# tulip-control/polytope

Hardware: AMD Instinct MI355X
Metric: LP solves/sec (batched Chebyshev + redundancy) (higher is better)
Workload: dtype f64

## Files before the change

### polytope_amd/csrc/plp_lane_lp.hpp

```cpp
#pragma once
#include <math.h>

#if defined(__HIPCC__)
#include "plp_common.hpp"
#define PLP_LANE_FN __device__ __forceinline__
#else
#define PLP_LANE_FN static inline
namespace plp {
enum : int { ST_OPT = 0, ST_ITER = 1, ST_INFEAS = 2, ST_UNBND = 3, ST_NUM = 4 };
constexpr int ST_RETRY = 5;
constexpr double TOL_D = 1e-9, TOL_PIV = 1e-7, DEGEN_EPS = 1e-12;
constexpr int BLAND_AFTER = 6;
}
#endif

namespace plp {
namespace lane {

constexpr int LANE_MAX_ITERS = 48;
constexpr double LANE_TOL_D = 1e-11, LANE_TOL_PIV = 1e-11;
constexpr double LANE_M_NOISE = 64 * 2.220446049250313e-16;

struct Lp3 {
    double x0, x1, x2;
    int w0, w1, w2;
    int nact;
    int status;
    int iters;
    int ndeg;
};

PLP_LANE_FN void cross3(double a0, double a1, double a2, double b0, double b1, double b2, double& e0, double& e1,
                        double& e2) {
    e0 = fma(a1, b2, -(a2 * b1));
    e1 = fma(a2, b0, -(a0 * b2));
    e2 = fma(a0, b1, -(a1 * b0));
}

PLP_LANE_FN double dot3(double a0, double a1, double a2, double b0, double b1, double b2) {
    return fma(a2, b2, fma(a1, b1, a0 * b0));
}

template <class AnyF>
PLP_LANE_FN void proj1(const double c0, const double c1, const double c2, const double cn1, const double n0, const double n1,
                       const double n2, const double nn, double& d0, double& d1, double& d2, double& scale, AnyF ANY) {
    const double cn = dot3(c0, c1, c2, n0, n1, n2);
    d0 = fma(cn, n0, -(nn * c0));
    d1 = fma(cn, n1, -(nn * c1));
    d2 = fma(cn, n2, -(nn * c2));
    scale = nn;
    const double pn1 = fabs(d0) + fabs(d1) + fabs(d2);
    const bool small = (pn1 > 0.0) & (pn1 < 1e-4 * (nn * cn1));
    if (ANY(small)) {
        const double np_ = dot3(n0, n1, n2, d0, d1, d2);
        const double q0 = fma(nn, d0, -(np_ * n0)), q1 = fma(nn, d1, -(np_ * n1)), q2 = fma(nn, d2, -(np_ * n2));
        d0 = small ? q0 : d0;
        d1 = small ? q1 : d1;
        d2 = small ? q2 : d2;
        scale = small ? nn * nn : nn;
    }
}

constexpr double LANE_PAIR_SIN2 = 1e-10;

template <class RowF, class RatioF, class Ratio0F, class AnyF>
PLP_LANE_FN void walk3(Lp3& S, const double c0, const double c1, const double c2, const bool go, RowF ROWS, RatioF RATIO,
                       Ratio0F RATIO0, AnyF ANY, const bool warm = false) {
    if (!warm) {
        S.x0 = S.x1 = S.x2 = 0.0;
        S.w0 = S.w1 = S.w2 = -1;
        S.nact = 0;
        S.iters = 0;
        S.ndeg = 0;
    }
    S.status = go ? -1 : ST_OPT;
    const double cn1 = fabs(c0) + fabs(c1) + fabs(c2);
    if (go && !(cn1 > 0.0)) S.status = ST_OPT;
    if (!warm && ANY(S.status < 0)) {
        const bool step = S.status < 0;
        const double d0 = -c0, d1 = -c1, d2 = -c2;
        const double tolp = LANE_TOL_PIV * cn1;
        double bs = 1.0, bd = 0.0;
        int bi = -1;
        RATIO0(d0, d1, d2, tolp, bs, bd, bi);
        if (step) {
            S.iters = 1;
            if (bi < 0) {
                S.status = ST_UNBND;
            } else {
                const double t = bs / bd;
                S.x0 = fma(t, d0, 0.0);
                S.x1 = fma(t, d1, 0.0);
                S.x2 = fma(t, d2, 0.0);
                S.w0 = bi;
                S.nact = 1;
                S.ndeg = (t * cn1 <= DEGEN_EPS) ? 1 : 0;
            }
        }
    }
    while (ANY(S.status < 0)) {
        const bool run = S.status < 0;
        double d0 = -c0, d1 = -c1, d2 = -c2;
        double n00 = 0, n01 = 0, n02 = 0, n10 = 0, n11 = 0, n12 = 0, n20 = 0, n21 = 0, n22 = 0;
        if (ANY(run && S.nact >= 1)) {
            if (S.nact >= 1) ROWS(S.w0, n00, n01, n02);
            if (S.nact >= 2) ROWS(S.w1, n10, n11, n12);
            if (S.nact >= 3) ROWS(S.w2, n20, n21, n22);
        }
        bool stalled = false;
        double dscale = cn1;
        if (S.nact == 1) {
            const double nn = dot3(n00, n01, n02, n00, n01, n02);
            double sc;
            proj1(c0, c1, c2, cn1, n00, n01, n02, nn, d0, d1, d2, sc, ANY);
            dscale = sc * cn1;
        } else if (S.nact == 2) {
            double e0, e1, e2;
            cross3(n00, n01, n02, n10, n11, n12, e0, e1, e2);
            const double ce = dot3(c0, c1, c2, e0, e1, e2);
            d0 = -(ce * e0);
            d1 = -(ce * e1);
            d2 = -(ce * e2);
            dscale = dot3(e0, e1, e2, e0, e1, e2) * cn1;
            const double nn0 = dot3(n00, n01, n02, n00, n01, n02), nn1 = dot3(n10, n11, n12, n10, n11, n12);
            if (run && !(dot3(e0, e1, e2, e0, e1, e2) > LANE_PAIR_SIN2 * nn0 * nn1)) S.status = ST_RETRY;
        } else if (S.nact == 3) {
            d0 = d1 = d2 = 0.0;
        }
        {
            const double dn1 = fabs(d0) + fabs(d1) + fabs(d2);
            stalled = !(dn1 > LANE_TOL_D * dscale);
        }
        if (ANY(S.status < 0 && stalled)) {
            if (S.status < 0 && stalled) {
                if (S.nact == 0) {
                    S.status = ST_OPT;
                } else if (S.nact == 1) {
                    const double cn = dot3(c0, c1, c2, n00, n01, n02);
                    if (cn <= 0.0) S.status = ST_OPT;
                    else { S.nact = 0; d0 = -c0; d1 = -c1; d2 = -c2; }
                } else if (S.nact == 2) {
                    const double g00 = dot3(n00, n01, n02, n00, n01, n02), g11 = dot3(n10, n11, n12, n10, n11, n12);
                    const double g01 = dot3(n00, n01, n02, n10, n11, n12);
                    const double r0 = -dot3(c0, c1, c2, n00, n01, n02), r1 = -dot3(c0, c1, c2, n10, n11, n12);
                    const double l0 = fma(r0, g11, -(r1 * g01)), l1 = fma(r1, g00, -(r0 * g01));
                    const double w0 = 0.5 * (1.0 + g00), w1 = 0.5 * (1.0 + g11);
                    const double tol0 = LANE_TOL_D * g11 * w0 * cn1, tol1 = LANE_TOL_D * g00 * w1 * cn1;
                    if (l0 >= -tol0 && l1 >= -tol1) S.status = ST_OPT;
                    else {
                        const bool drop0 = l0 * w0 < l1 * w1;
                        if (drop0) { S.w0 = S.w1; n00 = n10; n01 = n11; n02 = n12; }
                        S.nact = 1;
                        double sc;
                        proj1(c0, c1, c2, cn1, n00, n01, n02, dot3(n00, n01, n02, n00, n01, n02), d0, d1, d2, sc, [](bool q) { return q; });
                    }
                } else {
                    double u00, u01, u02, u10, u11, u12, u20, u21, u22;
                    cross3(n10, n11, n12, n20, n21, n22, u00, u01, u02);
                    cross3(n20, n21, n22, n00, n01, n02, u10, u11, u12);
                    cross3(n00, n01, n02, n10, n11, n12, u20, u21, u22);
                    const double det = dot3(n00, n01, n02, u00, u01, u02);
                    const double g00 = dot3(n00, n01, n02, n00, n01, n02), g11 = dot3(n10, n11, n12, n10, n11, n12);
                    const double g22 = dot3(n20, n21, n22, n20, n21, n22);
                    if (!(det * det > 1e-18 * (g00 * g11 * g22))) {
                        S.status = ST_RETRY;
                    } else {
                        const double sg = det > 0.0 ? 1.0 : -1.0;
                        const double l0 = -sg * dot3(c0, c1, c2, u00, u01, u02);
                        const double l1 = -sg * dot3(c0, c1, c2, u10, u11, u12);
                        const double l2 = -sg * dot3(c0, c1, c2, u20, u21, u22);
                        const double a0 = l0 * (0.5 * (1.0 + g00)), a1 = l1 * (0.5 * (1.0 + g11)), a2 = l2 * (0.5 * (1.0 + g22));
                        const double tol = LANE_TOL_D * fabs(det) * cn1;
                        if (a0 >= -tol && a1 >= -tol && a2 >= -tol) S.status = ST_OPT;
                        else {
                            int j = 0;
                            double am = a0;
                            if (a1 < am) { am = a1; j = 1; }
                            if (a2 < am) { am = a2; j = 2; }
                            double gg;
                            if (j == 0) { d0 = -sg * u00; d1 = -sg * u01; d2 = -sg * u02; S.w0 = S.w1; S.w1 = S.w2; gg = g11 * g22; }
                            else if (j == 1) { d0 = -sg * u10; d1 = -sg * u11; d2 = -sg * u12; S.w1 = S.w2; gg = g22 * g00; }
                            else { d0 = -sg * u20; d1 = -sg * u21; d2 = -sg * u22; gg = g00 * g11; }
                            S.nact = 2;
                            if (!(dot3(d0, d1, d2, d0, d1, d2) > LANE_PAIR_SIN2 * gg)) S.status = ST_RETRY;
                        }
                    }
                }
            }
        }
        const bool step = S.status < 0;
        const double dn1 = fabs(d0) + fabs(d1) + fabs(d2);
        const double tolp = LANE_TOL_PIV * dn1;
        double bs = 1.0, bd = 0.0;
        int bi = -1;
        if (ANY(step)) RATIO(d0, d1, d2, S.x0, S.x1, S.x2, tolp, bs, bd, bi);
        if (step) {
            ++S.iters;
            if (bi < 0) {
                S.status = ST_UNBND;
            } else {
                const double t = bs / bd;
                S.x0 = fma(t, d0, S.x0);
                S.x1 = fma(t, d1, S.x1);
                S.x2 = fma(t, d2, S.x2);
                if (S.nact == 0) S.w0 = bi;
                else if (S.nact == 1) S.w1 = bi;
                else S.w2 = bi;
                S.nact += 1;
                S.ndeg = (t * dn1 <= DEGEN_EPS) ? S.ndeg + 1 : 0;
                if (S.ndeg >= BLAND_AFTER || S.iters >= LANE_MAX_ITERS) S.status = ST_RETRY;
            }
        }
    }
}

template <class RowF, class RatioF, class AnyF>
PLP_LANE_FN void walk3(Lp3& S, const double c0, const double c1, const double c2, const bool go, RowF ROWS, RatioF RATIO,
                       AnyF ANY, const bool warm = false) {
    walk3(S, c0, c1, c2, go, ROWS, RATIO,
          [&](double d0, double d1, double d2, double tolp, double& bs, double& bd, int& bi) {
              RATIO(d0, d1, d2, 0.0, 0.0, 0.0, tolp, bs, bd, bi);
          },
          ANY, warm);
}

struct Lp4 {
    double x0, x1, x2, x3;
    int w0, w1, w2, w3;
    int nact, status, iters, ndeg;
};

PLP_LANE_FN double dot4(double a0, double a1, double a2, double a3, double b0, double b1, double b2, double b3) {
    return fma(a3, b3, fma(a2, b2, fma(a1, b1, a0 * b0)));
}

PLP_LANE_FN void gcross4(double p0, double p1, double p2, double p3, double q0, double q1, double q2, double q3, double r0,
                         double r1, double r2, double r3, double& e0, double& e1, double& e2, double& e3) {
    const double m01 = fma(q0, r1, -(q1 * r0)), m02 = fma(q0, r2, -(q2 * r0)), m03 = fma(q0, r3, -(q3 * r0));
    const double m12 = fma(q1, r2, -(q2 * r1)), m13 = fma(q1, r3, -(q3 * r1)), m23 = fma(q2, r3, -(q3 * r2));
    e0 = fma(p1, m23, fma(-p2, m13, p3 * m12));
    e1 = -fma(p0, m23, fma(-p2, m03, p3 * m02));
    e2 = fma(p0, m13, fma(-p1, m03, p3 * m01));
    e3 = -fma(p0, m12, fma(-p1, m02, p2 * m01));
}

template <class RowF, class RatioF, class AnyF>
PLP_LANE_FN void walk4(Lp4& S, const double c0, const double c1, const double c2, const double c3, const bool go, RowF ROWS,
                       RatioF RATIO, AnyF ANY) {
    S.x0 = S.x1 = S.x2 = S.x3 = 0.0;
    S.w0 = S.w1 = S.w2 = S.w3 = -1;
    S.nact = 0;
    S.iters = 0;
    S.ndeg = 0;
    S.status = go ? -1 : ST_OPT;
    const double cn1 = fabs(c0) + fabs(c1) + fabs(c2) + fabs(c3);
    if (go && !(cn1 > 0.0)) S.status = ST_OPT;
    while (ANY(S.status < 0)) {
        const bool run = S.status < 0;
        bool dropped = false;
        double d0 = -c0, d1 = -c1, d2 = -c2, d3 = -c3;
        double n00 = 0, n01 = 0, n02 = 0, n03 = 0, n10 = 0, n11 = 0, n12 = 0, n13 = 0;
        double n20 = 0, n21 = 0, n22 = 0, n23 = 0, n30 = 0, n31 = 0, n32 = 0, n33 = 0;
        if (ANY(run && S.nact >= 1)) {
            if (S.nact >= 1) ROWS(S.w0, n00, n01, n02, n03);
            if (S.nact >= 2) ROWS(S.w1, n10, n11, n12, n13);
            if (S.nact >= 3) ROWS(S.w2, n20, n21, n22, n23);
            if (S.nact >= 4) ROWS(S.w3, n30, n31, n32, n33);
        }
        const double g00 = dot4(n00, n01, n02, n03, n00, n01, n02, n03), g11 = dot4(n10, n11, n12, n13, n10, n11, n12, n13);
        const double g22 = dot4(n20, n21, n22, n23, n20, n21, n22, n23);
        const double g01 = dot4(n00, n01, n02, n03, n10, n11, n12, n13), g02 = dot4(n00, n01, n02, n03, n20, n21, n22, n23);
        const double g12 = dot4(n10, n11, n12, n13, n20, n21, n22, n23);
        const double r0 = dot4(c0, c1, c2, c3, n00, n01, n02, n03), r1 = dot4(c0, c1, c2, c3, n10, n11, n12, n13);
        const double r2 = dot4(c0, c1, c2, c3, n20, n21, n22, n23);
        double det = 1.0, m0 = 0.0, m1 = 0.0, m2 = 0.0;
        if (S.nact == 1) {
            det = g00;
            m0 = r0;
        } else if (S.nact == 2) {
            det = fma(g00, g11, -(g01 * g01));
            m0 = fma(r0, g11, -(r1 * g01));
            m1 = fma(r1, g00, -(r0 * g01));
            if (run && !(det > LANE_PAIR_SIN2 * g00 * g11)) S.status = ST_RETRY;
        } else if (S.nact == 3) {
            const double A00 = fma(g11, g22, -(g12 * g12)), A01 = fma(g02, g12, -(g01 * g22)), A02 = fma(g01, g12, -(g02 * g11));
            const double A11 = fma(g00, g22, -(g02 * g02)), A12 = fma(g01, g02, -(g00 * g12)), A22 = fma(g00, g11, -(g01 * g01));
            det = fma(g00, A00, fma(g01, A01, g02 * A02));
            m0 = fma(A00, r0, fma(A01, r1, A02 * r2));
            m1 = fma(A01, r0, fma(A11, r1, A12 * r2));
            m2 = fma(A02, r0, fma(A12, r1, A22 * r2));
            if (run && !(det > 1e-16 * g00 * g11 * g22)) S.status = ST_RETRY;
        }
        bool twice = false;
        if (S.nact == 3) {
            double e0, e1, e2, e3;
            gcross4(n00, n01, n02, n03, n10, n11, n12, n13, n20, n21, n22, n23, e0, e1, e2, e3);
            const double ce = dot4(c0, c1, c2, c3, e0, e1, e2, e3);
            d0 = -(ce * e0);
            d1 = -(ce * e1);
            d2 = -(ce * e2);
            d3 = -(ce * e3);
        } else if (S.nact >= 1 && S.nact <= 2) {
            d0 = fma(m1, n10, fma(m0, n00, -(det * c0)));
            d1 = fma(m1, n11, fma(m0, n01, -(det * c1)));
            d2 = fma(m1, n12, fma(m0, n02, -(det * c2)));
            d3 = fma(m1, n13, fma(m0, n03, -(det * c3)));
            if (S.nact == 1) {
                const double nd = dot4(n00, n01, n02, n03, d0, d1, d2, d3);
                d0 = fma(g00, d0, -(nd * n00));
                d1 = fma(g00, d1, -(nd * n01));
                d2 = fma(g00, d2, -(nd * n02));
                d3 = fma(g00, d3, -(nd * n03));
            } else {
                const double dn = fabs(d0) + fabs(d1) + fabs(d2) + fabs(d3);
                twice = (dn > 0.0) & (dn < 1e-4 * (det * cn1));
                if (ANY(run && twice)) {
                    const double s0 = dot4(d0, d1, d2, d3, n00, n01, n02, n03), s1 = dot4(d0, d1, d2, d3, n10, n11, n12, n13);
                    const double k0 = fma(s0, g11, -(s1 * g01)), k1 = fma(s1, g00, -(s0 * g01));
                    const double q0 = fma(det, d0, -fma(k1, n10, k0 * n00)), q1 = fma(det, d1, -fma(k1, n11, k0 * n01));
                    const double q2 = fma(det, d2, -fma(k1, n12, k0 * n02)), q3 = fma(det, d3, -fma(k1, n13, k0 * n03));
                    d0 = twice ? q0 : d0;
                    d1 = twice ? q1 : d1;
                    d2 = twice ? q2 : d2;
                    d3 = twice ? q3 : d3;
                }
            }
        } else if (S.nact == 4) {
            d0 = d1 = d2 = d3 = 0.0;
        }
        const double dscale = (S.nact >= 1 && S.nact <= 3) ? ((S.nact == 1 || twice) ? det * det : det) * cn1 : cn1;
        const bool stalled = !(fabs(d0) + fabs(d1) + fabs(d2) + fabs(d3) > LANE_TOL_D * dscale);
        if (ANY(S.status < 0 && stalled)) {
            if (S.status < 0 && stalled) {
                const double w0 = 0.5 * (1.0 + g00), w1 = 0.5 * (1.0 + g11), w2 = 0.5 * (1.0 + g22);
                if (S.nact == 0) {
                    S.status = ST_OPT;
                } else if (S.nact <= 3) {
                    const double tol = LANE_TOL_D * det * cn1;
                    double f0 = 0.0, f1 = 0.0, f2 = 0.0;
                    if (S.nact == 2) {
                        f0 = fabs(r0 * g11) + fabs(r1 * g01);
                        f1 = fabs(r1 * g00) + fabs(r0 * g01);
                    } else if (S.nact == 3) {
                        const double B00 = fabs(g11 * g22) + g12 * g12, B01 = fabs(g02 * g12) + fabs(g01 * g22), B02 = fabs(g01 * g12) + fabs(g02 * g11);
                        const double B11 = fabs(g00 * g22) + g02 * g02, B12 = fabs(g01 * g02) + fabs(g00 * g12), B22 = fabs(g00 * g11) + g01 * g01;
                        f0 = B00 * fabs(r0) + B01 * fabs(r1) + B02 * fabs(r2);
                        f1 = B01 * fabs(r0) + B11 * fabs(r1) + B12 * fabs(r2);
                        f2 = B02 * fabs(r0) + B12 * fabs(r1) + B22 * fabs(r2);
                    }
                    const double a0 = -m0 * w0, a1 = S.nact >= 2 ? -m1 * w1 : 0.0, a2 = S.nact >= 3 ? -m2 * w2 : 0.0;
                    const double t0 = fmax(tol, LANE_M_NOISE * f0 * w0), t1 = fmax(tol, LANE_M_NOISE * f1 * w1), t2 = fmax(tol, LANE_M_NOISE * f2 * w2);
                    if (a0 >= -t0 && a1 >= -t1 && a2 >= -t2) {
                        S.status = ST_OPT;
                    } else {
                        int j = 0;
                        double am = a0 + t0;
                        if (a1 + t1 < am) { am = a1 + t1; j = 1; }
                        if (a2 + t2 < am) { am = a2 + t2; j = 2; }
                        if (j == 0) S.w0 = S.w1;
                        if (j <= 1) S.w1 = S.w2;
                        S.nact -= 1;
                        dropped = true;
                    }
                } else {
                    const double g33 = dot4(n30, n31, n32, n33, n30, n31, n32, n33);
                    const double w3 = 0.5 * (1.0 + g33);
                    double am = 0.0, bd0 = 0.0, bd1 = 0.0, bd2 = 0.0, bd3 = 0.0, dj_abs = 0.0;
                    int jbest = -1;
                    bool all_ok = true, singular = false;
#define PLP_W4_VERTEX(J, P, Q, R, NJ0, NJ1, NJ2, NJ3, WJ)                                                          \
                    {                                                                                                   \
                        double u0, u1, u2, u3;                                                                          \
                        gcross4(P##0, P##1, P##2, P##3, Q##0, Q##1, Q##2, Q##3, R##0, R##1, R##2, R##3, u0, u1, u2, u3); \
                        const double dj = dot4(NJ0, NJ1, NJ2, NJ3, u0, u1, u2, u3);                                     \
                        const double sg = dj > 0.0 ? 1.0 : -1.0;                                                        \
                        const double lj = -sg * dot4(c0, c1, c2, c3, u0, u1, u2, u3);                                   \
                        const double aj = lj * (WJ);                                                                    \
                        dj_abs = fabs(dj);                                                                              \
                        singular = singular | !(dj * dj > 1e-18 * (g00 * g11 * g22 * g33));                            \
                        all_ok = all_ok & (aj >= -(LANE_TOL_D * dj_abs * cn1));                                              \
                        const bool better = (jbest < 0) | (aj < am);                                                    \
                        am = better ? aj : am;                                                                          \
                        jbest = better ? (J) : jbest;                                                                   \
                        bd0 = better ? -sg * u0 : bd0;                                                                  \
                        bd1 = better ? -sg * u1 : bd1;                                                                  \
                        bd2 = better ? -sg * u2 : bd2;                                                                  \
                        bd3 = better ? -sg * u3 : bd3;                                                                  \
                    }
                    PLP_W4_VERTEX(0, n1, n2, n3, n00, n01, n02, n03, w0)
                    PLP_W4_VERTEX(1, n0, n2, n3, n10, n11, n12, n13, w1)
                    PLP_W4_VERTEX(2, n0, n1, n3, n20, n21, n22, n23, w2)
                    PLP_W4_VERTEX(3, n0, n1, n2, n30, n31, n32, n33, w3)
#undef PLP_W4_VERTEX
                    if (singular) S.status = ST_RETRY;
                    else if (all_ok) S.status = ST_OPT;
                    else {
                        d0 = bd0; d1 = bd1; d2 = bd2; d3 = bd3;
                        if (jbest == 0) S.w0 = S.w1;
                        if (jbest <= 1) S.w1 = S.w2;
                        if (jbest <= 2) S.w2 = S.w3;
                        S.nact = 3;
                    }
                }
            }
        }
        if (dropped) {
            ++S.iters;
            if (S.iters >= LANE_MAX_ITERS) S.status = ST_RETRY;
        }
        const bool step = (S.status < 0) & !dropped;
        const double dn1 = fabs(d0) + fabs(d1) + fabs(d2) + fabs(d3);
        const double tolp = LANE_TOL_PIV * dn1;
        double bs = 1.0, bd = 0.0;
        int bi = -1;
        if (ANY(step)) RATIO(d0, d1, d2, d3, S.x0, S.x1, S.x2, S.x3, tolp, bs, bd, bi);
        if (step) {
            ++S.iters;
            if (bi < 0) {
                S.status = ST_UNBND;
            } else {
                const double t = bs / bd;
                S.x0 = fma(t, d0, S.x0);
                S.x1 = fma(t, d1, S.x1);
                S.x2 = fma(t, d2, S.x2);
                S.x3 = fma(t, d3, S.x3);
                if (S.nact == 0) S.w0 = bi;
                else if (S.nact == 1) S.w1 = bi;
                else if (S.nact == 2) S.w2 = bi;
                else S.w3 = bi;
                S.nact += 1;
                S.ndeg = (t * dn1 <= DEGEN_EPS) ? S.ndeg + 1 : 0;
                if (S.ndeg >= BLAND_AFTER || S.iters >= LANE_MAX_ITERS) S.status = ST_RETRY;
            }
        }
    }
}

PLP_LANE_FN void ratio_row4(const double a0, const double a1, const double a2, const double a3, const double beta, const int i,
                            const double d0, const double d1, const double d2, const double d3, const double x0,
                            const double x1, const double x2, const double x3, const double tolp, double& bs, double& bd,
                            int& bi) {
    const double ad = dot4(a0, a1, a2, a3, d0, d1, d2, d3);
    const double ax = dot4(a0, a1, a2, a3, x0, x1, x2, x3);
    const double sl = fmax(beta - ax, 0.0);
    const bool better = (ad > tolp) & (sl * bd < bs * ad);
    bs = better ? sl : bs;
    bd = better ? ad : bd;
    bi = better ? i : bi;
}

PLP_LANE_FN void ratio_row(const double a0, const double a1, const double a2, const double beta, const int i, const double d0,
                           const double d1, const double d2, const double x0, const double x1, const double x2,
                           const double tolp, double& bs, double& bd, int& bi) {
    const double ad = dot3(a0, a1, a2, d0, d1, d2);
    const double ax = dot3(a0, a1, a2, x0, x1, x2);
    const double sl = fmax(beta - ax, 0.0);
    const bool better = (ad > tolp) & (sl * bd < bs * ad);
    bs = better ? sl : bs;
    bd = better ? ad : bd;
    bi = better ? i : bi;
}

PLP_LANE_FN void ratio_row0(const double a0, const double a1, const double a2, const double beta, const int i, const double d0,
                            const double d1, const double d2, const double tolp, double& bs, double& bd, int& bi) {
    const double ad = dot3(a0, a1, a2, d0, d1, d2);
    const double sl = fmax(beta, 0.0);
    const bool better = (ad > tolp) & (sl * bd < bs * ad);
    bs = better ? sl : bs;
    bd = better ? ad : bd;
    bi = better ? i : bi;
}

#ifndef PLP_LANE_CH
#define PLP_LANE_CH 4
#endif

PLP_LANE_FN void latch_row(const bool elig, const bool closer, const double sl, const double ad, const int i, double& bs,
                           double& bd, int& bi) {
#if defined(__HIP_DEVICE_COMPILE__) && !defined(PLP_LANE_SELECT_LATCH)
    const unsigned long long mask = __builtin_amdgcn_ballot_w64(elig) & __builtin_amdgcn_ballot_w64(closer);
    unsigned long long saved;
    asm("s_and_saveexec_b64 %[sv], %[m]\n\t"
        "v_mov_b64 %[bs], %[sl]\n\t"
        "v_mov_b64 %[bd], %[ad]\n\t"
        "v_mov_b32 %[bi], %[i]\n\t"
        "s_mov_b64 exec, %[sv]"
        : [bs] "+v"(bs), [bd] "+v"(bd), [bi] "+v"(bi), [sv] "=&s"(saved)
        : [m] "s"(mask), [sl] "v"(sl), [ad] "v"(ad), [i] "s"(i)
        : "scc");
#else
    const bool better = elig & closer;
    bs = better ? sl : bs;
    bd = better ? ad : bd;
    bi = better ? i : bi;
#endif
}

PLP_LANE_FN double relax_row(const bool at, double beta) {
#if defined(__HIP_DEVICE_COMPILE__) && !defined(PLP_LANE_SELECT_LATCH)
    const unsigned long long mask = __builtin_amdgcn_ballot_w64(at);
    unsigned long long saved;
    asm("s_and_saveexec_b64 %[sv], %[m]\n\t"
        "v_add_f64 %[b], %[b], %[c]\n\t"
        "s_mov_b64 exec, %[sv]"
        : [b] "+v"(beta), [sv] "=&s"(saved)
        : [m] "s"(mask), [c] "s"(0.1)
        : "scc");
    return beta;
#else
    return at ? beta + 0.1 : beta;
#endif
}

enum : int { RATIO_WALK = 0, RATIO_FIRST = 1, RATIO_AXIS = 2 };

template <int D, int LS, int MODE, bool RELAX>
PLP_LANE_FN void ratio_rows(const double* pA, const double* pbeta, const int i0, const int cnt, const int krv,
                            const double (&dv)[4], const double (&xv)[4], const int kax, const double dk, const double tolp,
                            double& bs, double& bd, int& bi) {
    static_assert(D >= 1 && D <= 4 && (D < 4 || MODE == RATIO_WALK), "R^4 has no peeled first pass");
    const double* ra = pA + i0 * D * LS + (MODE == RATIO_AXIS ? kax * LS : 0);
    const double* rb = pbeta + i0 * LS;
    const int krel = krv - i0;
    int li = -1;
    for (int ch = 0; ch < cnt; ch += PLP_LANE_CH) {
#pragma unroll
        for (int r = 0; r < PLP_LANE_CH; ++r) {
            const double* a = ra + (r * D) * LS;
            double beta = rb[r * LS];
            if constexpr (RELAX) beta = relax_row(ch + r == krel, beta);
            double ad, sl;
            if constexpr (MODE == RATIO_AXIS) {
                ad = dk * a[0];
                sl = fmax(beta, 0.0);
            } else {
                const double a0 = a[0];
                const double a1 = D > 1 ? a[(D > 1 ? 1 : 0) * LS] : 0.0;
                const double a2 = D > 2 ? a[(D > 2 ? 2 : 0) * LS] : 0.0;
                if constexpr (D == 4) {
                    const double a3 = a[(D > 3 ? 3 : 0) * LS];
                    ad = dot4(a0, a1, a2, a3, dv[0], dv[1], dv[2], dv[3]);
                    sl = fmax(fma(-a3, xv[3], fma(-a2, xv[2], fma(-a1, xv[1], fma(-a0, xv[0], beta)))), 0.0);
                } else {
                    ad = dot3(a0, a1, a2, dv[0], dv[1], dv[2]);
                    sl = MODE == RATIO_FIRST ? fmax(beta, 0.0) : fmax(fma(-a2, xv[2], fma(-a1, xv[1], fma(-a0, xv[0], beta))), 0.0);
                }
            }
            latch_row(ad > tolp, sl * bd < bs * ad, sl, ad, ch + r, bs, bd, li);
        }
        ra += PLP_LANE_CH * D * LS;
        rb += PLP_LANE_CH * LS;
    }
    bi = li < 0 ? bi : li + i0;
}

template <int M, class RowF, class BetaF, class AnyF, class PassF>
PLP_LANE_FN void solve3(Lp3& S, const double c0, const double c1, const double c2, const bool go, RowF ROWS, BetaF BETA,
                        AnyF ANY, PassF PASS, const bool warm = false) {
    walk3(S, c0, c1, c2, go, ROWS,
          [&](double d0, double d1, double d2, double x0, double x1, double x2, double tolp, double& bs, double& bd, int& bi) {
              PASS();
#pragma unroll
              for (int i = 0; i < M; ++i) {
                  double a0, a1, a2;
                  ROWS(i, a0, a1, a2);
                  ratio_row(a0, a1, a2, BETA(i), i, d0, d1, d2, x0, x1, x2, tolp, bs, bd, bi);
              }
          },
          ANY, warm);
}

template <int M, class RowF, class BetaF, class AnyF>
PLP_LANE_FN void solve3(Lp3& S, const double c0, const double c1, const double c2, const bool go, RowF ROWS, BetaF BETA,
                        AnyF ANY, const bool warm = false) {
    solve3<M>(S, c0, c1, c2, go, ROWS, BETA, ANY, [] {}, warm);
}

}
}
```

Baseline: 14.16 billion.

## Peel facet and edge passes out of the lane LP walk loop

Adds specialised facet and edge passes that run after the first ratio step of a cold walk. Lanes that sit on one or two constraints take their next pivots without going through the general branchy loop, which is meant to cut divergence and wasted work across the wavefront. Row loads in the general loop become unconditional, using index 0 as a dummy. This trades extra memory reads for less branching. Optional tally hooks for counting walk events are also added and compile to nothing by default.

```diff
diff --git a/polytope_amd/csrc/plp_lane_lp.hpp b/polytope_amd/csrc/plp_lane_lp.hpp
--- a/polytope_amd/csrc/plp_lane_lp.hpp
+++ b/polytope_amd/csrc/plp_lane_lp.hpp
@@ -63,6 +63,98 @@
 
 constexpr double LANE_PAIR_SIN2 = 1e-10;
 
+enum : int {
+    WE_OPT1 = 0, WE_OPT2, WE_OPT3,
+    WE_UNBND,
+    WE_RETRY_PAIR, WE_RETRY_TRIPLE, WE_RETRY_DEGEN,
+    WE_DROP2, WE_DROP3,
+    WE_PASS_FACET, WE_PASS_EDGE, WE_PASS_GENERAL,
+    WE_COUNT
+};
+#ifndef PLP_LANE_TALLY
+#define PLP_LANE_TALLY(e) ((void)0)
+#endif
+
+template <bool CAPS>
+PLP_LANE_FN void step3(Lp3& S, const bool step, const double d0, const double d1, const double d2, const double dn1,
+                       const double bs, const double bd, const int bi, const int slot) {
+    static_assert(BLAND_AFTER > 3 && LANE_MAX_ITERS > 3, "passes 2 and 3 of a walk from the centre reach neither cap");
+    if (step) {
+        ++S.iters;
+        if (bi < 0) {
+            S.status = ST_UNBND;
+            PLP_LANE_TALLY(WE_UNBND);
+        } else {
+            const double t = bs / bd;
+            S.x0 = fma(t, d0, S.x0);
+            S.x1 = fma(t, d1, S.x1);
+            S.x2 = fma(t, d2, S.x2);
+            if (slot == 0) S.w0 = bi;
+            else if (slot == 1) S.w1 = bi;
+            else S.w2 = bi;
+            S.nact = slot + 1;
+            S.ndeg = (t * dn1 <= DEGEN_EPS) ? S.ndeg + 1 : 0;
+            if (CAPS && (S.ndeg >= BLAND_AFTER || S.iters >= LANE_MAX_ITERS)) {
+                S.status = ST_RETRY;
+                PLP_LANE_TALLY(WE_RETRY_DEGEN);
+            }
+        }
+    }
+}
+
+#ifndef PLP_LANE_PLAIN_WALK
+
+template <class RowF, class RatioF, class AnyF>
+PLP_LANE_FN void facet_pass3(Lp3& S, const double c0, const double c1, const double c2, const double cn1, RowF ROWS,
+                             RatioF RATIO, AnyF ANY) {
+    const bool on = S.status < 0 && S.nact == 1;
+    double n0, n1, n2;
+    ROWS(on ? S.w0 : 0, n0, n1, n2);
+    const double nn = dot3(n0, n1, n2, n0, n1, n2);
+    double d0, d1, d2, sc;
+    proj1(c0, c1, c2, cn1, n0, n1, n2, nn, d0, d1, d2, sc, ANY);
+    const double dn1 = fabs(d0) + fabs(d1) + fabs(d2);
+    const bool step = on && (dn1 > LANE_TOL_D * (sc * cn1));
+    if (ANY(step)) {
+        double bs = 1.0, bd = 0.0;
+        int bi = -1;
+        RATIO(d0, d1, d2, S.x0, S.x1, S.x2, LANE_TOL_PIV * dn1, bs, bd, bi);
+        if (step) PLP_LANE_TALLY(WE_PASS_FACET);
+        step3<false>(S, step, d0, d1, d2, dn1, bs, bd, bi, 1);
+    }
+}
+
+template <class RowF, class RatioF, class AnyF>
+PLP_LANE_FN void edge_pass3(Lp3& S, const double c0, const double c1, const double c2, const double cn1, RowF ROWS,
+                            RatioF RATIO, AnyF ANY) {
+    const bool on = S.status < 0 && S.nact == 2;
+    double n00, n01, n02, n10, n11, n12;
+    ROWS(on ? S.w0 : 0, n00, n01, n02);
+    ROWS(on ? S.w1 : 0, n10, n11, n12);
+    double e0, e1, e2;
+    cross3(n00, n01, n02, n10, n11, n12, e0, e1, e2);
+    const double ce = dot3(c0, c1, c2, e0, e1, e2);
+    const double d0 = -(ce * e0), d1 = -(ce * e1), d2 = -(ce * e2);
+    const double ee = dot3(e0, e1, e2, e0, e1, e2);
+    const double nn0 = dot3(n00, n01, n02, n00, n01, n02), nn1 = dot3(n10, n11, n12, n10, n11, n12);
+    const bool edge = ee > LANE_PAIR_SIN2 * nn0 * nn1;
+    if (on && !edge) {
+        S.status = ST_RETRY;
+        PLP_LANE_TALLY(WE_RETRY_PAIR);
+        PLP_LANE_TALLY(WE_PASS_EDGE);
+    }
+    const double dn1 = fabs(d0) + fabs(d1) + fabs(d2);
+    const bool step = on && edge && (dn1 > LANE_TOL_D * (ee * cn1));
+    if (ANY(step)) {
+        double bs = 1.0, bd = 0.0;
+        int bi = -1;
+        RATIO(d0, d1, d2, S.x0, S.x1, S.x2, LANE_TOL_PIV * dn1, bs, bd, bi);
+        if (step) PLP_LANE_TALLY(WE_PASS_EDGE);
+        step3<false>(S, step, d0, d1, d2, dn1, bs, bd, bi, 2);
+    }
+}
+#endif
+
 template <class RowF, class RatioF, class Ratio0F, class AnyF>
 PLP_LANE_FN void walk3(Lp3& S, const double c0, const double c1, const double c2, const bool go, RowF ROWS, RatioF RATIO,
                        Ratio0F RATIO0, AnyF ANY, const bool warm = false) {
@@ -87,6 +179,7 @@
             S.iters = 1;
             if (bi < 0) {
                 S.status = ST_UNBND;
+                PLP_LANE_TALLY(WE_UNBND);
             } else {
                 const double t = bs / bd;
                 S.x0 = fma(t, d0, 0.0);
@@ -98,15 +191,26 @@
             }
         }
     }
+#ifndef PLP_LANE_PLAIN_WALK
+    if (!warm && ANY(S.status < 0 && S.nact == 1)) facet_pass3(S, c0, c1, c2, cn1, ROWS, RATIO, ANY);
+    if (!warm && ANY(S.status < 0 && S.nact == 2)) edge_pass3(S, c0, c1, c2, cn1, ROWS, RATIO, ANY);
+#endif
     while (ANY(S.status < 0)) {
         const bool run = S.status < 0;
+        if (run) PLP_LANE_TALLY(WE_PASS_GENERAL);
         double d0 = -c0, d1 = -c1, d2 = -c2;
         double n00 = 0, n01 = 0, n02 = 0, n10 = 0, n11 = 0, n12 = 0, n20 = 0, n21 = 0, n22 = 0;
+#ifdef PLP_LANE_PLAIN_WALK
         if (ANY(run && S.nact >= 1)) {
             if (S.nact >= 1) ROWS(S.w0, n00, n01, n02);
             if (S.nact >= 2) ROWS(S.w1, n10, n11, n12);
             if (S.nact >= 3) ROWS(S.w2, n20, n21, n22);
         }
+#else
+        ROWS(S.nact >= 1 ? S.w0 : 0, n00, n01, n02);
+        ROWS(S.nact >= 2 ? S.w1 : 0, n10, n11, n12);
+        ROWS(S.nact >= 3 ? S.w2 : 0, n20, n21, n22);
+#endif
         bool stalled = false;
         double dscale = cn1;
         if (S.nact == 1) {
@@ -123,7 +227,10 @@
             d2 = -(ce * e2);
             dscale = dot3(e0, e1, e2, e0, e1, e2) * cn1;
             const double nn0 = dot3(n00, n01, n02, n00, n01, n02), nn1 = dot3(n10, n11, n12, n10, n11, n12);
-            if (run && !(dot3(e0, e1, e2, e0, e1, e2) > LANE_PAIR_SIN2 * nn0 * nn1)) S.status = ST_RETRY;
+            if (run && !(dot3(e0, e1, e2, e0, e1, e2) > LANE_PAIR_SIN2 * nn0 * nn1)) {
+                S.status = ST_RETRY;
+                PLP_LANE_TALLY(WE_RETRY_PAIR);
+            }
         } else if (S.nact == 3) {
             d0 = d1 = d2 = 0.0;
         }
@@ -137,7 +244,7 @@
                     S.status = ST_OPT;
                 } else if (S.nact == 1) {
                     const double cn = dot3(c0, c1, c2, n00, n01, n02);
-                    if (cn <= 0.0) S.status = ST_OPT;
+                    if (cn <= 0.0) { S.status = ST_OPT; PLP_LANE_TALLY(WE_OPT1); }
                     else { S.nact = 0; d0 = -c0; d1 = -c1; d2 = -c2; }
                 } else if (S.nact == 2) {
                     const double g00 = dot3(n00, n01, n02, n00, n01, n02), g11 = dot3(n10, n11, n12, n10, n11, n12);
@@ -146,8 +253,9 @@
                     const double l0 = fma(r0, g11, -(r1 * g01)), l1 = fma(r1, g00, -(r0 * g01));
                     const double w0 = 0.5 * (1.0 + g00), w1 = 0.5 * (1.0 + g11);
                     const double tol0 = LANE_TOL_D * g11 * w0 * cn1, tol1 = LANE_TOL_D * g00 * w1 * cn1;
-                    if (l0 >= -tol0 && l1 >= -tol1) S.status = ST_OPT;
+                    if (l0 >= -tol0 && l1 >= -tol1) { S.status = ST_OPT; PLP_LANE_TALLY(WE_OPT2); }
                     else {
+                        PLP_LANE_TALLY(WE_DROP2);
                         const bool drop0 = l0 * w0 < l1 * w1;
                         if (drop0) { S.w0 = S.w1; n00 = n10; n01 = n11; n02 = n12; }
                         S.nact = 1;
@@ -164,6 +272,7 @@
                     const double g22 = dot3(n20, n21, n22, n20, n21, n22);
                     if (!(det * det > 1e-18 * (g00 * g11 * g22))) {
                         S.status = ST_RETRY;
+                        PLP_LANE_TALLY(WE_RETRY_TRIPLE);
                     } else {
                         const double sg = det > 0.0 ? 1.0 : -1.0;
                         const double l0 = -sg * dot3(c0, c1, c2, u00, u01, u02);
@@ -171,8 +280,9 @@
                         const double l2 = -sg * dot3(c0, c1, c2, u20, u21, u22);
                         const double a0 = l0 * (0.5 * (1.0 + g00)), a1 = l1 * (0.5 * (1.0 + g11)), a2 = l2 * (0.5 * (1.0 + g22));
                         const double tol = LANE_TOL_D * fabs(det) * cn1;
-                        if (a0 >= -tol && a1 >= -tol && a2 >= -tol) S.status = ST_OPT;
+                        if (a0 >= -tol && a1 >= -tol && a2 >= -tol) { S.status = ST_OPT; PLP_LANE_TALLY(WE_OPT3); }
                         else {
+                            PLP_LANE_TALLY(WE_DROP3);
                             int j = 0;
                             double am = a0;
                             if (a1 < am) { am = a1; j = 1; }
@@ -182,7 +292,10 @@
                             else if (j == 1) { d0 = -sg * u10; d1 = -sg * u11; d2 = -sg * u12; S.w1 = S.w2; gg = g22 * g00; }
                             else { d0 = -sg * u20; d1 = -sg * u21; d2 = -sg * u22; gg = g00 * g11; }
                             S.nact = 2;
-                            if (!(dot3(d0, d1, d2, d0, d1, d2) > LANE_PAIR_SIN2 * gg)) S.status = ST_RETRY;
+                            if (!(dot3(d0, d1, d2, d0, d1, d2) > LANE_PAIR_SIN2 * gg)) {
+                                S.status = ST_RETRY;
+                                PLP_LANE_TALLY(WE_RETRY_PAIR);
+                            }
                         }
                     }
                 }
@@ -194,23 +307,7 @@
         double bs = 1.0, bd = 0.0;
         int bi = -1;
         if (ANY(step)) RATIO(d0, d1, d2, S.x0, S.x1, S.x2, tolp, bs, bd, bi);
-        if (step) {
-            ++S.iters;
-            if (bi < 0) {
-                S.status = ST_UNBND;
-            } else {
-                const double t = bs / bd;
-                S.x0 = fma(t, d0, S.x0);
-                S.x1 = fma(t, d1, S.x1);
-                S.x2 = fma(t, d2, S.x2);
-                if (S.nact == 0) S.w0 = bi;
-                else if (S.nact == 1) S.w1 = bi;
-                else S.w2 = bi;
-                S.nact += 1;
-                S.ndeg = (t * dn1 <= DEGEN_EPS) ? S.ndeg + 1 : 0;
-                if (S.ndeg >= BLAND_AFTER || S.iters >= LANE_MAX_ITERS) S.status = ST_RETRY;
-            }
-        }
+        step3<true>(S, step, d0, d1, d2, dn1, bs, bd, bi, S.nact);
     }
 }
 
```

New measurement: 14.66 billion (median of 6 runs). 3.6% higher.
